# KT19/distributed-training-compare-jax

Measured on AMD Instinct MI355X. Metric: avg step time (ms) + tokens/sec, GPT-2-small DP/TP/PP at 1/2/4/8 MI355X, higher is better.
Workload: dtype bf16; 1 GPU; model=gpt2-small-124M (d768 L12 H12 F3072 T1024 V50258), global_batch=8, seq_len=1024, parallelism=dp1, capture_comms=True, hipgraph=True, backend=nccl, world_size=1, graph_segments=1, eager_collectives=0

## Files before the change

### distributed_training_compare_jax_amd/csrc/gemm.hip

```cpp
#include "common.h"
#include "gemm_plan.h"
#include <algorithm>
#include <cstdlib>
#include <type_traits>

namespace {

constexpr int NT = 256;

template <int R, int BK, bool KMAJ>
struct Tile {
  static constexpr int LD = KMAJ ? (BK + 16) : (R + 16);
  static constexpr int ROWS = KMAJ ? R : BK;
  static constexpr int ELEMS = ROWS * LD;
  static constexpr int CHUNKS = R * BK / 8;
  static constexpr int PER_THREAD = CHUNKS / NT;
  static_assert(CHUNKS % NT == 0, "tile too small for 256 threads");

  __device__ __forceinline__ static void load(u32x4 (&reg)[PER_THREAD], __amdgpu_buffer_rsrc_t rs, long ld, int r0,
                                              int k0, int tid) {
#pragma unroll
    for (int i = 0; i < PER_THREAD; ++i) {
      int c = tid + i * NT;
      long off;
// ... 1494 lines not shown
    case 3: P8_VMCNT(3); break;
    case 4: P8_VMCNT(4); break;
    case 5: P8_VMCNT(5); break;
    case 6: P8_VMCNT(6); break;
    case 8: P8_VMCNT(8); break;
    case 9: P8_VMCNT(9); break;
    case 10: P8_VMCNT(10); break;
    case 11: P8_VMCNT(11); break;
    case 12: P8_VMCNT(12); break;
    case 15: P8_VMCNT(15); break;
    case 16: P8_VMCNT(16); break;
    case 18: P8_VMCNT(18); break;
    default: P8_VMCNT(0); break;
  }
}

template <int B, int E, typename F>
__device__ __forceinline__ void static_for(F&& f) {
  if constexpr (B < E) {
    f(std::integral_constant<int, B>{});
    static_for<B + 1, E>(f);
  }
}

template <int EPI, bool OUTF32>
__device__ __forceinline__ void n8_frag_out(const Epi& e, int m, int n, f32x4 v, f32x4 bias, bf16x4 aux) {
  float o[4];
#pragma unroll
  for (int r = 0; r < 4; ++r) o[r] = v[r] + bias[r];
  if (EPI == EPI_DGELU) {
#pragma unroll
    for (int r = 0; r < 4; ++r) o[r] *= (float)aux[r];
  }
  if (OUTF32) {
    *(f32x4*)((float*)e.C + (long)m * e.ldc + n) = f32x4{o[0], o[1], o[2], o[3]};
    return;
  }
  bf16x4 ob, gb;
#pragma unroll
  for (int r = 0; r < 4; ++r) {
    if (EPI == EPI_GELU) {
      float gv, dgv;
      gelu_tanh_and_grad_f(o[r], gv, dgv);
      ob[r] = f2bf(dgv);
      gb[r] = f2bf(gv);
    } else {
      ob[r] = f2bf(o[r]);
    }
  }
  *(bf16x4*)((bf16*)e.C + (long)m * e.ldc + n) = ob;
  if (EPI == EPI_GELU) *(bf16x4*)((bf16*)e.aux_out + (long)m * e.ldc + n) = gb;
}

template <int CB, int NS, bool AK, bool BKM, int EPI, bool OUTF32>
__global__ void __launch_bounds__(NT2, 1)
gemm8n_kernel(const bf16* __restrict__ A, long lda, const bf16* __restrict__ B, long ldb, int M, int N, int K,
              int tiles_m, int tiles_n, int gm, Epi e) {
  static_assert(NS >= 3, "stage t+1 must be issued before the phase-0 wait of step t");
  constexpr int CA = 2, TM = 4, TN = CB, BN = 64 * CB, D = NS - 1, PIECES = CA + CB;
  constexpr int SIMG = PIECES * P8_CHUNK;
  __shared__ __attribute__((aligned(16))) bf16 smem[NS * SIMG];
  const int tid = threadIdx.x, lane = tid & 63, wave = tid >> 6;
  const int wr = wave >> 2, wc = wave & 3;
  const int ntiles = tiles_m * tiles_n;
  const int G = gridDim.x;
  const int bl = xcd_remap(blockIdx.x, G);
  const int nk = K / 64;
  DTC_ASSERT(nk >= 1);
  const int nr = bl < ntiles ? (ntiles - bl + G - 1) / G : 0;
  const int S = nr * nk;
  if (S == 0) return;
  auto origin = [&](int r, int& m0, int& n0) {
    const int tile = bl + r * G;
    const int grp = tile / (gm * tiles_n), in_g = tile % (gm * tiles_n);
    const int gm_eff = min(gm, tiles_m - grp * gm);
    m0 = (grp * gm + in_g % gm_eff) * 128;
    n0 = (in_g / gm_eff) * BN;
  };

  f32x4 acc[TN][TM];
#pragma unroll
  for (int i = 0; i < TN; ++i)
#pragma unroll
    for (int j = 0; j < TM; ++j) acc[i][j] = f32x4{0.f, 0.f, 0.f, 0.f};

  constexpr bool OVL = EPI == EPI_STORE || EPI == EPI_GELU;
  constexpr int NFRAG = TN * TM, NPEEL = OVL ? NFRAG / 4 : 0;
  f32x4 pacc[TN][TM], pbias[TN];
  bool pend = false;
  int em0 = 0, en0 = 0;
  const int g4e = 4 * (lane >> 4);
  auto epi_frag = [&](auto F) {
    constexpr int f = decltype(F)::value, i = f / TM, j = f % TM;
    const int m = em0 + wr * 64 + j * 16 + (lane & 15);
    const int n = en0 + wc * 16 * TN + i * 16 + g4e;
    if (m < M) n8_frag_out<EPI, OUTF32>(e, m, n, pacc[i][j], pbias[i], bf16x4{});
  };
  int cm0, cn0;
  origin(0, cm0, cn0);
  DTC_ASSERT(nk >= NPEEL);

  auto imgA = [&](int s) { return smem + (s % NS) * SIMG; };
  auto imgB = [&](int s) { return smem + (s % NS) * SIMG + CA * P8_CHUNK; };
  int pr = 0, pk = 0;
  const bf16* srcA[CA];
  const bf16* srcB[CB];
  long offA = 0, offB = 0;
  const long stepA = AK ? 64 : 64 * lda, stepB = BKM ? 64 : 64 * ldb;
  auto set_src = [&](int r) {
    int m0, n0;
    origin(r, m0, n0);
#pragma unroll
    for (int q = 0; q < CA; ++q) srcA[q] = p8_src<AK>(A, lda, m0, M, q, wave, lane);
#pragma unroll
    for (int q = 0; q < CB; ++q) srcB[q] = p8_src<BKM>(B, ldb, n0, N, q, wave, lane);
    offA = offB = 0;
  };
  set_src(0);
  auto advance = [&]() {
    offA += stepA;
    offB += stepB;
    if (++pk == nk) {
      pk = 0;
      ++pr;
      if (pr < nr) set_src(pr);
    }
  };
  auto dmaA = [&](int s, int q) { p8_dma_at(srcA[q] + offA, imgA(s), q, wave); };
  auto dmaB = [&](int s, int q) { p8_dma_at(srcB[q] + offB, imgB(s), q, wave); };

  const int npro = min(D, S);
  for (int s = 0; s < npro; ++s) {
#pragma unroll
    for (int q = 0; q < CB; ++q) dmaB(s, q);
#pragma unroll
    for (int q = 0; q < CA; ++q) dmaA(s, q);
    advance();
  }
  n8_vmcnt((npro - 1) * PIECES);
  __builtin_amdgcn_s_barrier();
  if (wr == 1) __builtin_amdgcn_s_barrier();

  int t = 0;
  bf16x8 fb[TN][2], fa[2][2];
  auto kstep = [&](auto SLc) {
    constexpr int SL = decltype(SLc)::value;
    const bf16* sA = imgA(t);
    const bf16* sB = imgB(t);
    const bool issue = t + D < S;
#pragma unroll
    for (int p = 0; p < 2; ++p) {
      if (p == 0) {
#pragma unroll
        for (int i = 0; i < TN; ++i)
#pragma unroll
          for (int kk = 0; kk < 2; ++kk) fb[i][kk] = p8_frag<BKM>(sB, TN * wc + i, kk, lane);
      }
#pragma unroll
      for (int jj = 0; jj < 2; ++jj)
#pragma unroll
        for (int kk = 0; kk < 2; ++kk) fa[jj][kk] = p8_frag<AK>(sA, 4 * wr + 2 * p + jj, kk, lane);
      if (issue) {
        if (p == 0) {
#pragma unroll
          for (int q = 0; q < CB; ++q) dmaB(t + D, q);
        } else {
#pragma unroll
          for (int q = 0; q < CA; ++q) dmaA(t + D, q);
          advance();
        }
      }
      __builtin_amdgcn_s_barrier();
      asm volatile("s_waitcnt lgkmcnt(0)" ::: "memory");
#pragma unroll
      for (int jj = 0; jj < 2; ++jj)
#pragma unroll
        for (int kk = 0; kk < 2; ++kk) asm volatile("" : "+v"(fa[jj][kk]));
#pragma unroll
      for (int i = 0; i < TN; ++i)
#pragma unroll
        for (int kk = 0; kk < 2; ++kk) asm volatile("" : "+v"(fb[i][kk]));
      __builtin_amdgcn_s_setprio(1);
#pragma unroll
      for (int kk = 0; kk < 2; ++kk)
#pragma unroll
        for (int i = 0; i < TN; ++i)
#pragma unroll
          for (int jj = 0; jj < 2; ++jj)
            acc[i][2 * p + jj] = __builtin_amdgcn_mfma_f32_16x16x32_bf16(fb[i][kk], fa[jj][kk], acc[i][2 * p + jj], 0, 0, 0);
      __builtin_amdgcn_s_setprio(0);
      if constexpr (SL >= 0) {
        if (pend) {
          if (p == 0) {
            epi_frag(std::integral_constant<int, 4 * SL>{});
            epi_frag(std::integral_constant<int, 4 * SL + 1>{});
          } else {
            epi_frag(std::integral_constant<int, 4 * SL + 2>{});
            epi_frag(std::integral_constant<int, 4 * SL + 3>{});
          }
        }
      }
      if (p == 0 && t + 1 < S) {
        if (t + D < S) {
          vmcnt_c<(D - 2) * PIECES + CB>();
        } else {
          const int full = max(0, min(t + D - 1, S - 1) - (t + 1));
          n8_vmcnt(full * PIECES);
        }
      }
      __builtin_amdgcn_s_barrier();
    }
    ++t;
  };
  for (int cr = 0; cr < nr; ++cr) {
    static_for<0, NPEEL>([&](auto sl) { kstep(sl); });
    for (int k = NPEEL; k < nk; ++k) kstep(std::integral_constant<int, -1>{});
    const int m0 = cm0, n0 = cn0;
    if (cr + 1 < nr) origin(cr + 1, cm0, cn0);
    const int g4 = 4 * (lane >> 4);
    if constexpr (OVL) {
#pragma unroll
      for (int i = 0; i < TN; ++i) {
        pbias[i] = e.bias ? *(const f32x4*)(e.bias + n0 + wc * 16 * TN + i * 16 + g4) : f32x4{0.f, 0.f, 0.f, 0.f};
#pragma unroll
        for (int j = 0; j < TM; ++j) pacc[i][j] = acc[i][j];
      }
      em0 = m0;
      en0 = n0;
      pend = true;
    } else if constexpr (EPI == EPI_NONE) {
#pragma unroll
      for (int i = 0; i < TN; ++i)
#pragma unroll
        for (int j = 0; j < TM; ++j) asm volatile("" ::"v"(acc[i][j]));
    } else {
#pragma unroll
      for (int i = 0; i < TN; ++i)
#pragma unroll
        for (int j = 0; j < TM; ++j) {
          const int m = m0 + wr * 64 + j * 16 + (lane & 15);
          const int n = n0 + wc * 16 * TN + i * 16 + g4;
          if (m < M && n < N) epilogue_store<EPI, OUTF32>(e, m, n, acc[i][j]);
        }
    }
#pragma unroll
    for (int i = 0; i < TN; ++i)
#pragma unroll
      for (int j = 0; j < TM; ++j) acc[i][j] = f32x4{0.f, 0.f, 0.f, 0.f};
  }
  if constexpr (OVL) static_for<0, NFRAG>([&](auto f) { epi_frag(f); });
  if (wr == 0) __builtin_amdgcn_s_barrier();
}

__device__ __forceinline__ bf16x8 ce_colsum_frag(const bf16* img, int r0, int vt, int lane) {
  const int g = lane >> 4, li = lane & 15, q = li >> 2, pp = li & 3;
  const int row = r0 + 4 * g + q;
  const int ch = 2 * vt + (pp >> 1);
  const bf16* p0 = img + row * 64 + ((ch ^ ((row >> 1) & 7)) << 3) + (pp & 1) * 4;
  const s16x4 lo = ds_tr16_asm(p0), hi = ds_tr16_asm(p0 + 16 * 64);
  return __builtin_bit_cast(bf16x8, __builtin_shufflevector(lo, hi, 0, 1, 2, 3, 4, 5, 6, 7));
}

struct CeDgradArgs {
  const bf16* logits; long ldl;
  const float* lse; const int* labels; int vocab_start, n_valid; float scale;
  const bf16* wt; long ldw;
  bf16* dlogits; long ldd;
  float* colpart;
  float* slab;
  int M, N, K, tiles_m, tiles_n, gm, split, kps;
};

__global__ void __launch_bounds__(NT2, 1) ce_dgrad256_kernel(CeDgradArgs a) {
  constexpr int TM = 8, TN = 4;
  __shared__ __attribute__((aligned(16))) bf16 smem[4 * IMG];
  const int tid = threadIdx.x, lane = tid & 63, wave = tid >> 6;
  const int wm = wave & 1, wn = wave >> 1;
  const int ntiles = a.tiles_m * a.tiles_n;
  const int lid = xcd_remap(blockIdx.x, ntiles * a.split);
  const int tile = lid % ntiles, z = lid / ntiles;
  const int grp = tile / (a.gm * a.tiles_n), in_g = tile % (a.gm * a.tiles_n);
  const int gm_eff = min(a.gm, a.tiles_m - grp * a.gm);
  const int tm_idx = grp * a.gm + in_g % gm_eff, tn_idx = in_g / gm_eff;
  const int m0 = tm_idx * BIG, n0 = tn_idx * BIG;
  DTC_ASSERT(tm_idx >= 0 && tn_idx >= 0 && z >= 0 && m0 < a.M && n0 < a.N);
  const int kbeg = z * a.kps;
  const int nk = min(a.kps, a.K - kbeg) / 64;
// ... 643 lines not shown
  if constexpr (V::epi == EPI_STORE && V::f32) {
    if (p.sub == 3) {
      const int tn3 = a.N / 192;
      hipLaunchKernelGGL((gemm8p_kernel<V::AK, V::BKM, V::epi, V::f32, 3>), dim3(tiles_m * tn3 * split), dim3(NT2), 0, st,
                         (const bf16*)a.A, a.lda, (const bf16*)a.B, a.ldb, a.M, a.N, a.K, tiles_m, tn3,
                         gm_round32(tiles_m, tn3), split, kps, (float*)a.workspace, e);
      DTC_CHECK_LAUNCH();
      note_launch(gp::FAM_BIG, BIG, 192, split, 3, 0, a.layout, V::epi);
      return finish_splitk(a, split, st);
    }
  }
  const int gm = tiles_n <= 16 ? gm_round32(tiles_m, tiles_n) : wide_gm(tiles_m);
  hipLaunchKernelGGL((gemm8p_kernel<V::AK, V::BKM, V::epi, V::f32>), dim3(tiles_m * tiles_n * split), dim3(NT2), 0, st,
                     (const bf16*)a.A, a.lda, (const bf16*)a.B, a.ldb, a.M, a.N, a.K, tiles_m, tiles_n, gm, split,
                     kps, (float*)a.workspace, e);
  DTC_CHECK_LAUNCH();
  note_launch(gp::FAM_BIG, BIG, BIG, split, 4, 0, a.layout, V::epi);
  return finish_splitk(a, split, st);
}

template <class V, int CB2>
int launch_r8_cb(const GemmArgs& a, const gp::GemmPlan& p, hipStream_t st) {
  const Epi e = make_epi(a, 0);
  R8Args r;
  r.A = (const bf16*)a.A; r.lda = a.lda; r.B = (const bf16*)a.B; r.ldb = a.ldb;
  r.M = a.M; r.N = a.N; r.K = a.K; r.n_split = p.aux;
  r.tm = a.M / BIG;
  r.tn1 = r.n_split / BIG;
  r.nb1 = r.tm * r.tn1;
  r.gm1 = r.tn1 > 0 ? gm_round32(r.tm, r.tn1) : 1;
  r.tn2 = (a.N - r.n_split) / (64 * CB2);
  r.gm2 = gm_round32(r.tm, std::max(1, r.tn2));
  r.ilv = g_knobs.r8_ilv && r.nb1 >= 2 && r.tm * r.tn2 >= 2;
  const int grid = r.nb1 + r.tm * r.tn2;
  hipLaunchKernelGGL((gemm8r_kernel<V::AK, V::BKM, V::epi, V::f32, CB2>), dim3(grid), dim3(NT2), 0, st, r, e);
  DTC_CHECK_LAUNCH();
  note_launch(gp::FAM_R8, BIG, 64 * CB2, 1, CB2, r.n_split, a.layout, V::epi);
  return 0;
}

template <class V>
int launch_r8(const GemmArgs& a, const gp::GemmPlan& p, hipStream_t st) {
  if (p.sub == 4) return launch_r8_cb<V, 4>(a, p, st);
  if (p.sub == 2) return launch_r8_cb<V, 2>(a, p, st);
  return launch_r8_cb<V, 1>(a, p, st);
}

template <class V, int CB>
int launch_n8_cb(const GemmArgs& a, hipStream_t st) {
  const Epi e = make_epi(a, 0);
  const int tiles_m = (a.M + 127) / 128, tiles_n = a.N / (64 * CB);
  constexpr int NS = CB == 3 ? 4 : 3;
  const int grid = std::min(tiles_m * tiles_n, cu_count());
  hipLaunchKernelGGL((gemm8n_kernel<CB, NS, V::AK, V::BKM, V::epi, V::f32>), dim3(grid), dim3(NT2), 0, st,
                     (const bf16*)a.A, a.lda, (const bf16*)a.B, a.ldb, a.M, a.N, a.K, tiles_m, tiles_n,
                     gm_n8(tiles_m, tiles_n), e);
  DTC_CHECK_LAUNCH();
  note_launch(gp::FAM_N8, 128, 64 * CB, 1, CB, 0, a.layout, V::epi);
  return 0;
}

template <class V>
int launch_n8(const GemmArgs& a, const gp::GemmPlan& p, hipStream_t st) {
  return p.sub == 3 ? launch_n8_cb<V, 3>(a, st) : launch_n8_cb<V, 4>(a, st);
}

template <class V, int CFG>
int launch_w(const GemmArgs& a, int split, hipStream_t st) {
  constexpr gp::WTile T = gp::W_TILES[CFG];
  const int tiles_m = (a.M + T.bm - 1) / T.bm, tiles_n = (a.N + T.bn - 1) / T.bn;
  const Epi e = make_epi(a, tiles_n * T.wgn);
  const int nk = a.K / 64;
  const int kps = ((nk + split - 1) / split) * 64;
  hipLaunchKernelGGL((gemm_dmaw_kernel<T.bm, T.bn, T.stages, T.wgm, T.wgn, V::AK, V::BKM, V::epi, V::f32>),
                     dim3(tiles_m * tiles_n * split), dim3(64 * T.wgm * T.wgn), 0, st, (const bf16*)a.A, a.lda,
                     (const bf16*)a.B, a.ldb, a.M, a.N, a.K, tiles_m, tiles_n, gm_xcd_share(tiles_m, tiles_n), split, kps,
                     (float*)a.workspace, e);
  DTC_CHECK_LAUNCH();
  note_launch(gp::FAM_DMAW, T.bm, T.bn, split, T.stages, T.wgm * 10 + T.wgn, a.layout, V::epi);
  return finish_splitk(a, split, st);
}

template <class V, int CFG>
int launch_w_if(const GemmArgs& a, const gp::GemmPlan& p, hipStream_t st) {
  if constexpr (gp::dmaw_cfg_has(CFG, V::layout, V::epi, V::f32))
    if (p.bm == gp::W_TILES[CFG].bm && p.bn == gp::W_TILES[CFG].bn) return launch_w<V, CFG>(a, p.split, st);
  return NOT_INSTANTIATED;
}

template <class V>
int launch_dmaw(const GemmArgs& a, const gp::GemmPlan& p, hipStream_t st) {
  int r = launch_w_if<V, gp::W_256x128>(a, p, st);
  if (r == NOT_INSTANTIATED) r = launch_w_if<V, gp::W_128x64>(a, p, st);
  if (r == NOT_INSTANTIATED) r = launch_w_if<V, gp::W_64x128>(a, p, st);
  if (r == NOT_INSTANTIATED) r = launch_w_if<V, gp::W_128x128>(a, p, st);
  return r;
}

int launch(const gp::GemmPlan& p, const GemmArgs& a, hipStream_t st) {
  return with_variant(a.layout, p.epi, p.f32, [&](auto v) {
    using V = decltype(v);
    constexpr int L = V::layout, E = V::epi;
    constexpr bool F = V::f32;
    switch (p.family) {
      case gp::FAM_R8: if constexpr (gp::r8_has(L, E, F)) return launch_r8<V>(a, p, st); break;
      case gp::FAM_N8: if constexpr (gp::n8_has(L, E, F)) return launch_n8<V>(a, p, st); break;
      case gp::FAM_DMAW: return launch_dmaw<V>(a, p, st);
      case gp::FAM_BIG: if constexpr (gp::big_has(L, E, F)) return launch_big<V>(a, p, st); break;
      case gp::FAM_REG:
// ... 123 lines not shown
  if (a->M <= 0 || a->M % 128 || a->N % 256 || a->N > 1024 || a->K <= 0 || a->K % 64) return 1400;
  if (a->lda % 8 || a->ldb % 8) return 1400;
  if (!a->sync || !a->step || !a->gamma || !a->err || !a->C || !a->y || !a->mean || !a->rstd) return 1401;
  if (a->bwd ? (!a->x || !a->part || a->nslab < 2 || a->nslab > 3) : (!a->resid || !a->beta)) return 1402;
  Epi e{};
  e.M = a->M; e.N = a->N; e.C = a->C; e.ldc = a->N; e.bias = a->bwd ? nullptr : a->bias;
  e.aux = a->resid; e.ldaux = a->N; e.alpha = 1.f;
  e.ln.gamma = a->gamma; e.ln.beta = a->beta; e.ln.y = (bf16*)a->y; e.ln.mean = a->mean; e.ln.rstd = a->rstd;
  e.ln.x = a->x; e.ln.part = a->part; e.ln.nslab = a->nslab; e.ln.eps = a->eps;
  e.ln.sync = a->sync; e.ln.step = a->step; e.ln.site = a->site; e.ln.nsites = a->nsites; e.ln.err = a->err;
  const int tiles_m = a->M / 128, tiles_n = a->N / 64;
  const dim3 grid(tiles_m * tiles_n), block(512);
  if (a->bwd)
    hipLaunchKernelGGL((gemm_dmaw_kernel<128, 64, 4, 4, 2, true, true, EPI_LN_BWD, true>), grid, block, 0, st,
                       (const bf16*)a->A, a->lda, (const bf16*)a->B, a->ldb, a->M, a->N, a->K, tiles_m, tiles_n, tiles_m,
                       1, a->K, nullptr, e);
  else
    hipLaunchKernelGGL((gemm_dmaw_kernel<128, 64, 4, 4, 2, true, true, EPI_RESID_LN, true>), grid, block, 0, st,
                       (const bf16*)a->A, a->lda, (const bf16*)a->B, a->ldb, a->M, a->N, a->K, tiles_m, tiles_n, tiles_m,
                       1, a->K, nullptr, e);
  DTC_CHECK_LAUNCH();
  note_launch(gp::FAM_LN, 128, 64, 1, a->bwd ? 1 : 0, 0, 0, a->bwd ? EPI_LN_BWD : EPI_RESID_LN);
  return 0;
}

long dtc_gemm_ln_sync_words(int M, int N) { return (long)M * (N / 32) + (long)(M / 128) * (N / 64); }

int dtc_lmhead_nparts(int M, int N, int K) {
  const gp::GemmPlan p = plan_query(0, M, N, K, EPI_LMHEAD, false, false);
  if (p.bn == BIG || gp::big_split(0, M, N, K, g_knobs)) return ((N + 255) / 256) * 4;
  return ((N + 127) / 128) * 2;
}

int dtc_gemm_wgrad_split(int M, int N, int K, int has_db) {
  return plan_query(2, M, N, K, EPI_STORE, true, has_db != 0).split;
}

int dtc_gemm_wgrad_fuses_colsum(int M, int N, int K) {
  return plan_query(2, M, N, K, EPI_STORE, true, true).err != 1009;
}

long dtc_gemm_workspace_bytes(int layout, int M, int N, int K) {
  const int bs = gp::big_split(layout, M, N, K, g_knobs);
  int split = bs ? bs : gp::reg_plan(M, N, K, layout == 2 ? 1 : (layout == 1 ? 2 : 0), g_knobs).split;
  if (layout == 2 && !bs) split = std::max(split, gp::dmaw_plan(2, M, N, K, EPI_STORE, true, false, g_knobs).split);
  return split > 1 ? (long)split * M * N * 4 : 0;
}

int dtc_gemm_set_wgrad256(int on) { return set_knob(g_knobs.wgrad256, on); }
int dtc_gemm_set_n8(int mask) { return set_knob(g_knobs.n8_mask, mask); }
int dtc_gemm_set_big_cb3(int on) { return set_knob(g_knobs.big_cb3, on); }
int dtc_gemm_set_n8_mink(int k) { return set_knob(g_knobs.n8_mink, k); }
int dtc_gemm_set_n8_cb(int cb) { return set_knob(g_knobs.n8_cb, cb); }
int dtc_gemm_set_r8(int mask) { return set_knob(g_knobs.r8_mask, mask); }
int dtc_gemm_set_r8_ilv(int on) { return set_knob(g_knobs.r8_ilv, on); }

int dtc_wg_entry_bytes() { return (int)sizeof(WgEntry); }
int dtc_wg_max() { return WG_MAX; }
int dtc_wg_batch_bytes() { return (int)sizeof(WgBatch); }

int dtc_wgrad_group(const WgBatch* in, hipStream_t st) {
  DTC_HOST_CHECK(in && in->n >= 1 && in->n <= WG_MAX && in->K >= 64 && in->K % 64 == 0);
  WgBatch b = *in;
  int t = 0;
  for (int i = 0; i < b.n; ++i) {
    WgEntry& w = b.e[i];
    DTC_HOST_CHECK(w.A && w.B && w.C && w.M >= 8 && w.N >= 8 && w.M % 8 == 0 && w.N % 8 == 0);
    DTC_HOST_CHECK(((unsigned long)w.A % 16) == 0 && ((unsigned long)w.B % 16) == 0 && ((unsigned long)w.C % 16) == 0);
    w.tile0 = t;
    t += ((w.M + BIG - 1) / BIG) * ((w.N + BIG - 1) / BIG);
    w.nfast = g_knobs.wg_nfast && w.M >= 2 * w.N;
  }
  b.ntiles = t;
  int tail = 0, split = 0;
  const int cus = cu_count();
  if (in->tail_slab && in->tail_split > 0 && cus > 0 && t > cus) {
    tail = t % cus;
    split = in->tail_split > 1 ? in->tail_split : std::max(2, std::min(4, tail > 0 ? cus / tail : 0));
    bool ok = tail > 0 && b.K % (64 * split) == 0 && (long)tail * split <= 2L * cus &&
              (long)tail * split * BIG * BIG <= in->tail_cap;
    for (int i = 0; ok && i < b.n; ++i) {
      const WgEntry& w = b.e[i];
      const int end = w.tile0 + ((w.M + BIG - 1) / BIG) * ((w.N + BIG - 1) / BIG);
      if (end > t - tail && w.cs) ok = false;
    }
    if (!ok) tail = split = 0;
  }
  b.tail_tiles = tail;
  b.tail_split = split > 1 ? split : 1;
  if (!tail) b.tail_slab = nullptr;
  hipLaunchKernelGGL(gemm8p_group_kernel, dim3(t - tail + tail * b.tail_split), dim3(NT2), 0, st, b);
  DTC_CHECK_LAUNCH();
  note_launch(gp::FAM_WGROUP, BIG, BIG, b.tail_split, tail, t, 2, EPI_STORE);
  if (tail) {
    hipLaunchKernelGGL(wg_tail_reduce, dim3(tail * 8), dim3(WGT_THREADS), 0, st, b);
    DTC_CHECK_LAUNCH();
  }
  return 0;
}

int dtc_gemm_last_launch(int* out) {
  const LastLaunch l = g_last;
  out[0] = l.family; out[1] = l.bm; out[2] = l.bn; out[3] = l.split;
  out[4] = l.sub; out[5] = l.aux; out[6] = l.layout; out[7] = l.epi;
  return 0;
}
// ... 3 lines not shown
```

### distributed_training_compare_jax_amd/csrc/gemm_plan.h

```cpp
#pragma once
#include <algorithm>
#include <climits>
#include <cstdlib>

namespace gp {

enum { EPI_STORE = 0, EPI_RESID = 1, EPI_GELU = 2, EPI_DGELU = 3, EPI_LMHEAD = 4, EPI_LMHEAD_EVAL = 7 };
constexpr int BIG = 256;

enum {
  FAM_NONE = 0,
  FAM_REG = 1,
  FAM_DMA64 = 2,
  FAM_DMAW = 3,
  FAM_BIG = 4,
  FAM_R8 = 5,
  FAM_N8 = 6,
  FAM_PAIR = 7,
  FAM_WGROUP = 8,
  FAM_CE_DGRAD = 9,
  FAM_LN = 10,
  FAM_COUNT = 11,
};

struct Knobs {
  int dma_fwd64 = 1;
  int wgrad_blocks_128 = 256;
  int wgrad_blocks_64 = 512;
  int wide_gm = 3;
  int wgrad_cs256 = 1;
  int wgrad256 = 1;
  int gemm256 = 7;
  int big_min_tiles = 512;
  int big_tail = 64;
  int big_cb3 = 1;
  int r8_mask = 5;
  int r8_ilv = 1;
  int n8_mask = 3;
  int n8_cb = 0;
  int n8_mink = 1024;
  int w8_mode = 1;
  int wg_nfast = 1;
};

inline int env_int(const char* value, int dflt) { return value ? atoi(value) : dflt; }

inline Knobs knobs_from_env() {
  Knobs k;
  k.dma_fwd64 = env_int(getenv("DTC_GEMM_DMA"), k.dma_fwd64);
  k.wgrad_blocks_128 = env_int(getenv("DTC_WGRAD_BLOCKS"), k.wgrad_blocks_128);
  k.wgrad_blocks_64 = env_int(getenv("DTC_WGRAD_BLOCKS"), k.wgrad_blocks_64);
  k.wide_gm = env_int(getenv("DTC_WIDE_GM"), k.wide_gm);
  k.wgrad_cs256 = env_int(getenv("DTC_WGRAD_CS256"), k.wgrad_cs256);
  k.wgrad256 = env_int(getenv("DTC_WGRAD256"), k.wgrad256);
  k.gemm256 = env_int(getenv("DTC_GEMM256"), k.gemm256);
  k.big_min_tiles = env_int(getenv("DTC_BIG_MIN_TILES"), k.big_min_tiles);
  k.big_tail = env_int(getenv("DTC_BIG_TAIL"), k.big_tail);
  k.big_cb3 = env_int(getenv("DTC_BIG_CB3"), k.big_cb3);
  k.r8_mask = env_int(getenv("DTC_GEMM8R"), k.r8_mask);
  k.r8_ilv = env_int(getenv("DTC_R8_ILV"), k.r8_ilv);
  k.n8_mask = env_int(getenv("DTC_GEMM8N"), k.n8_mask);
  k.n8_cb = env_int(getenv("DTC_N8_CB"), k.n8_cb);
  k.n8_mink = env_int(getenv("DTC_N8_MINK"), k.n8_mink);
  k.w8_mode = env_int(getenv("DTC_GEMM_W8"), k.w8_mode);
  k.wg_nfast = env_int(getenv("DTC_WG_NFAST"), k.wg_nfast);
  return k;
}

struct Problem {
  int layout, M, N, K;
  int epi;
  bool f32;
  bool has_bias, has_colsum;
  bool unit_ab;
  bool eval_ok;
  long ws_bytes;
};

struct GemmPlan {
  int err = 0;
  int family = FAM_NONE;
  int bm = 0, bn = 0;
  int bk = 64;
  int split = 1;
  int sub = 0, aux = 0;
  int epi = 0;
  bool f32 = false;
};

inline GemmPlan reg_plan(int M, int N, int K, int allow_split, const Knobs& k) {
  GemmPlan p;
  p.family = FAM_REG;
  p.bm = p.bn = 128;
  if (K % 64) {
    p.bm = p.bn = 64;
    p.bk = 32;
    return p;
  }
  const int nk = K / 64;
  const long t128 = (long)((M + 127) / 128) * ((N + 127) / 128);
  if (allow_split && K >= 8192 && t128 >= 32) {
    p.split = (int)std::max(1L, std::min((long)nk / 64, (512 + t128 - 1) / t128));
    return p;
  }
  if (allow_split == 1 && t128 < 256) {
    while (t128 * p.split < k.wgrad_blocks_128 && nk / (p.split * 2) >= 8) p.split *= 2;
    return p;
  }
  if (t128 >= 256) return p;
  p.bm = p.bn = 64;
  const long t64 = (long)((M + 63) / 64) * ((N + 63) / 64);
  if (allow_split == 1)
    while (t64 * p.split < k.wgrad_blocks_64 && nk / (p.split * 2) >= 4) p.split *= 2;
  return p;
}

// ... 263 lines not shown
```

### distributed_training_compare_jax_amd/models/gpt.py

```python

from __future__ import annotations

import contextlib
from dataclasses import dataclass
from typing import Dict, Optional, Tuple

import torch

from ..config.schema import ModelConfig
from ..ops import attention as A
from ..ops import embedding as E
from ..ops import gemm as G
from ..ops import layernorm as LN
from ..ops import fp8 as F8
from ..ops import mxfp8 as MX
from ..ops import ln_fused as LF
from ..ops import xent as X
from ..ops.reduce import GradReducer
from .params import head_split
from ..parallel.buffers import FlatParams


import os as _os

_CE_FUSED_MODE = _os.environ.get("DTC_CE_FUSED", "auto")


def _ce_fused(tokens: int, d: int) -> bool:
    if _CE_FUSED_MODE == "auto":
        return tokens * d <= 4096 * 512
    return _CE_FUSED_MODE == "1"
_CE_CHUNK = int(_os.environ.get("DTC_CE_CHUNK", "0"))
_ADD_LN = _os.environ.get("DTC_ADD_LN", "1") == "1"
_FWD_BF16 = _os.environ.get("DTC_FWD_BF16", "0") == "1"
_RED_BATCH_LAYERS = _os.environ.get("DTC_RED_BATCH_LAYERS", "1") == "1"
if _CE_CHUNK < 0 or _CE_CHUNK % 256:
    raise ValueError(f"DTC_CE_CHUNK={_CE_CHUNK}: must be 0 (off) or a positive multiple of 256 vocab columns")



_HEAD_BF16_MAXK = 16384


class _Staged:

    __slots__ = ("rows", "cols", "device")

    def __init__(self, rows: int, cols: int, device):
        self.rows, self.cols, self.device = rows, cols, device

class NoComm:

    size = 1
    rank = 0

    def all_reduce_(self, t):
        return t

    def all_gather_stack(self, t):
        return t.unsqueeze(0)


@dataclass
class StageLayout:
    layers: range
    has_embed: bool
    has_head: bool
    head_part: Tuple[int, int] = (0, 1)


class GPTStage:

    def __init__(self, cfg: ModelConfig, flat: FlatParams, layout: StageLayout, tp=None,
                 dropout_seed: int = 0, act_dtype: torch.dtype = torch.bfloat16):
        self.cfg = cfg
        dev = torch.device(flat.device)
        layer_bytes = 4 * (4 * cfg.d_model * cfg.d_model + 2 * cfg.d_model * cfg.d_ff)
        self.red = GradReducer(dev, arena_mb=max(512, (32 * layer_bytes // 3) >> 20)) if dev.type == "cuda" else None
        self._bias_fused = set()
        self.param_ready: Dict = {}
        self.flat = flat
        self.layout = layout
        self.tp = tp if tp is not None else NoComm()
        self.seed = int(dropout_seed)
        self.act_dtype = act_dtype
        D, H = cfg.d_model, cfg.n_heads
# ... 183 lines not shown
            y1q = MX.quant_mxfp8(y1)
        qkv = MX.linear_mxfp8(y1q, f.wmx(p + "qkv.w"), f.p(p + "qkv.b"), out_dtype=act)
        o, lse = A.attn_fwd(qkv.view(batch, T, -1), self.heads_local)
        o = o.view(batch * T, -1)
        oq = MX.quant_mxfp8(o)
        if _ADD_LN:
            br = MX.linear_mxfp8(oq, f.wmx(p + "out.w"), f.p(p + "out.b"), out_dtype=self._branch_dtype)
            x2, (y2, mu2, rs2), y2q = MX.add_layernorm_fwd_mx(br, x, f.p(p + "ln2.g"), f.p(p + "ln2.b"), self.eps, act)
        else:
            x2 = MX.linear_resid_mxfp8(oq, f.wmx(p + "out.w"), f.p(p + "out.b"), x)
            (y2, mu2, rs2), y2q = MX.layernorm_fwd_mx(x2, f.p(p + "ln2.g"), f.p(p + "ln2.b"), self.eps, act)
        u, gact, gq = MX.linear_gelu_mxfp8(y2q, f.wmx(p + "fc1.w"), f.p(p + "fc1.b"), out_dtype=act, quant_out=True)
        nxt = f"h.{l + 1}.ln1" if (l + 1) in self.layout.layers else ("lnf" if self.layout.has_head else None)
        if _ADD_LN and nxt is not None:
            br = MX.linear_mxfp8(gq, f.wmx(p + "fc2.w"), f.p(p + "fc2.b"), out_dtype=self._branch_dtype)
            if nxt == "lnf":
                x3, ctx["lnf_pre"] = LN.add_layernorm_fwd(br, x2, f.p("lnf.g"), f.p("lnf.b"), self.eps, act)
            else:
                x3, ctx[("ln1", l + 1)], ctx[("ln1_mx", l + 1)] = MX.add_layernorm_fwd_mx(
                    br, x2, f.p(nxt + ".g"), f.p(nxt + ".b"), self.eps, act)
        else:
            x3 = MX.linear_resid_mxfp8(gq, f.wmx(p + "fc2.w"), f.p(p + "fc2.b"), x2)
        ctx[l] = (x, y1, mu1, rs1, qkv, o, lse, x2, y2, mu2, rs2, u, gact, batch)
        return x3

    def block_forward(self, l: int, x: torch.Tensor, batch: int, ctx: Dict) -> torch.Tensor:
        if self.sp:
            return self._block_forward_sp(l, x, batch, ctx)
        if self.mx:
            return self._block_forward_mx(l, x, batch, ctx)
        self._await_params(l)
        f, p = self.flat, f"h.{l}."
        tp = self.tp
        lead = tp.rank == 0
        T = x.shape[0] // batch
        pre = ctx.pop(("ln1", l), None)
        if pre is None:
            pre = LN.layernorm_fwd(x, f.p(p + "ln1.g"), f.p(p + "ln1.b"), self.eps, self.act_dtype)
        y1, mu1, rs1 = pre
        fp8 = self.fp8
        if fp8:
            qkv = F8.linear_fp8(F8.quant_e4m3(y1), f.w8(p + "qkv.w"), f.p(p + "qkv.b"), out_dtype=self.act_dtype)
        else:
            qkv = G.linear(y1, f.w(p + "qkv.w"), f.p(p + "qkv.b"))
        o, lse = A.attn_fwd(qkv.view(batch, T, -1), self.heads_local)
        o = o.view(batch * T, -1)
        oq = F8.quant_e4m3(o) if fp8 else None
        if self._fuse_fwd:
            x2, (y2, mu2, rs2) = LF.linear_resid_ln(o, f.w(p + "out.w"), f.p(p + "out.b"), x, f.p(p + "ln2.g"),
                                                    f.p(p + "ln2.b"), self.eps, self.ln_sync, self._ln_site(l, 0, False))
        elif self.tp_bf16:
            x2 = self._row_parallel(o, p + "out.w", resid=x, bias=f.p(p + "out.b"))
            y2, mu2, rs2 = LN.layernorm_fwd(x2, f.p(p + "ln2.g"), f.p(p + "ln2.b"), self.eps, self.act_dtype)
        elif tp.size == 1 and _ADD_LN:
            br = (F8.linear_fp8(oq, f.w8(p + "out.w"), f.p(p + "out.b"), out_dtype=self._branch_dtype) if fp8 else
                  G.linear(o, f.w(p + "out.w"), f.p(p + "out.b"), out_dtype=self._branch_dtype))
            x2, (y2, mu2, rs2) = LN.add_layernorm_fwd(br, x, f.p(p + "ln2.g"), f.p(p + "ln2.b"), self.eps,
                                                      self.act_dtype)
        else:
            if fp8:
                x2 = F8.linear_resid_fp8(oq, f.w8(p + "out.w"), f.p(p + "out.b"), x)
            else:
                x2 = G.linear_resid(o, f.w(p + "out.w"), f.p(p + "out.b") if lead else None, x if lead else None)
            tp.all_reduce_(x2)
            y2, mu2, rs2 = LN.layernorm_fwd(x2, f.p(p + "ln2.g"), f.p(p + "ln2.b"), self.eps, self.act_dtype)
        if fp8:
            u, gact = F8.linear_gelu_fp8(F8.quant_e4m3(y2), f.w8(p + "fc1.w"), f.p(p + "fc1.b"), out_dtype=self.act_dtype)
            gq = F8.quant_e4m3(gact)
        else:
            u, gact = G.linear_gelu(y2, f.w(p + "fc1.w"), f.p(p + "fc1.b"))
        nxt = f"h.{l + 1}.ln1" if (l + 1) in self.layout.layers else ("lnf" if self.layout.has_head else None)
        if self._fuse_fwd and nxt is not None:
            x3, pre_next = LF.linear_resid_ln(gact, f.w(p + "fc2.w"), f.p(p + "fc2.b"), x2, f.p(nxt + ".g"),
                                              f.p(nxt + ".b"), self.eps, self.ln_sync, self._ln_site(l, 1, False))
            ctx[("ln1", l + 1) if nxt != "lnf" else "lnf_pre"] = pre_next
        elif tp.size == 1 and _ADD_LN and nxt is not None and not self.tp_bf16:
            br = (F8.linear_fp8(gq, f.w8(p + "fc2.w"), f.p(p + "fc2.b"), out_dtype=self._branch_dtype) if fp8 else
                  G.linear(gact, f.w(p + "fc2.w"), f.p(p + "fc2.b"), out_dtype=self._branch_dtype))
            x3, pre_next = LN.add_layernorm_fwd(br, x2, f.p(nxt + ".g"), f.p(nxt + ".b"), self.eps, self.act_dtype)
            ctx[("ln1", l + 1) if nxt != "lnf" else "lnf_pre"] = pre_next
        elif self.tp_bf16:
            x3 = self._row_parallel(gact, p + "fc2.w", resid=x2, bias=f.p(p + "fc2.b"))
        elif fp8:
            x3 = F8.linear_resid_fp8(gq, f.w8(p + "fc2.w"), f.p(p + "fc2.b"), x2)
        else:
            x3 = G.linear_resid(gact, f.w(p + "fc2.w"), f.p(p + "fc2.b") if lead else None, x2 if lead else None)
            tp.all_reduce_(x3)
        ctx[l] = (x, y1, mu1, rs1, qkv, o, lse, x2, y2, mu2, rs2, u, gact, batch)
        return x3

    def block_backward(self, l: int, ctx: Dict, dx3: torch.Tensor, dx3_c: torch.Tensor, beta: float, dx_hook=None):
        if self.sp:
            return self._block_backward_sp(l, ctx, dx3, dx3_c, beta, dx_hook)
        f, p = self.flat, f"h.{l}."
        x, y1, mu1, rs1, qkv, o, lse, x2, y2, mu2, rs2, u, gact, batch = ctx.pop(l)
        T = x.shape[0] // batch
        red = self.red
        fc2b_fused = l in self._bias_fused
        self._bias_fused.discard(l)
        self._beta = beta
        if self._defer_wg:
            wt2 = f.wt(p + "fc2.w")
            du = (G.matmul_nt_dgelu(dx3_c, wt2, u) if wt2 is not None
                  else G.matmul_nn_dgelu(dx3_c, f.w(p + "fc2.w"), u))
            self._wg(dx3_c, gact, p + "fc2")
            if not fc2b_fused:
                G.colsum(dx3, f.g(p + "fc2.b"), beta, red=red)
        else:
            du = G.linear_backward(dx3_c, f.w(p + "fc2.w"), gact, f.g(p + "fc2.w"), beta, red=red, dgelu_u=u,
                                   wt=f.wt(p + "fc2.w"))
            if not fc2b_fused:
                G.colsum(dx3, f.g(p + "fc2.b"), beta, red=red)
        wt1 = f.wt(p + "fc1.w")
        if self._fuse_bwd and wt1 is not None:
            dx2, dx2_c = LF.dgrad_ln_bwd(du, wt1, x2, f.p(p + "ln2.g"), mu2, rs2, dx3, f.g(p + "ln2.g"),
                                         f.g(p + "ln2.b"), beta, dbias=f.g(p + "out.b"), red=red,
                                         sync=self.ln_sync, site=self._ln_site(l, 0, True))
            self._wg(du, y2, p + "fc1", bias=True)
        else:
            dy2 = self._tp_reduce(self._dgrad_wgrad(du, p + "fc1", y2, beta, red, pair=False))
            dx2, dx2_c = self._ln_bwd(dy2, x2, p + "ln2", mu2, rs2, dx3, beta, bias_grad=p + "out.b")
        wto = f.wt(p + "out.w")
        if wto is not None:
            do = G.linear(dx2_c, wto)
            self._wg(dx2_c, o, p + "out")
        elif self._defer_wg:
            do = G.matmul_nn(dx2_c, f.w(p + "out.w"), out_dtype=self.act_dtype)
            self._wg(dx2_c, o, p + "out")
        else:
# ... 423 lines not shown
```

### distributed_training_compare_jax_amd/ops/_native.py

```python

from __future__ import annotations

import ctypes
import os
import threading

import torch

_LIB = None
_LOCK = threading.Lock()
LIB_NAME = "_dtc_kernels.so"
PKG_DIR = os.path.dirname(os.path.dirname(os.path.abspath(__file__)))
LIB_PATH = os.environ.get("DTC_KERNEL_LIB") or os.path.join(PKG_DIR, LIB_NAME)

c_int = ctypes.c_int
c_long = ctypes.c_long
c_float = ctypes.c_float
c_vp = ctypes.c_void_p


class GemmArgs(ctypes.Structure):

    _fields_ = [
        ("layout", c_int),
# ... 29 lines not shown
        ("C", c_vp),
        ("bias", c_vp), ("resid", c_vp), ("gamma", c_vp), ("beta", c_vp),
        ("y", c_vp), ("mean", c_vp), ("rstd", c_vp),
        ("x", c_vp), ("part", c_vp), ("nslab", c_int),
        ("eps", c_float),
        ("sync", c_vp), ("step", c_vp), ("site", c_int), ("nsites", c_int),
        ("err", c_vp),
    ]


class WgEntry(ctypes.Structure):

    _fields_ = [("A", c_vp), ("B", c_vp), ("C", c_vp), ("cs", c_vp), ("M", c_int), ("N", c_int),
                ("tile0", c_int), ("nfast", c_int)]


WG_MAX = 64


class WgBatch(ctypes.Structure):
    _fields_ = [("n", c_int), ("K", c_int), ("beta", c_float), ("ntiles", c_int), ("sq", c_vp),
                ("tail_tiles", c_int), ("tail_split", c_int), ("tail_slab", c_vp), ("tail_cap", c_long),
                ("e", WgEntry * WG_MAX)]


EPI_STORE = 0
EPI_RESID = 1
EPI_GELU = 2
EPI_DGELU = 3
EPI_LMHEAD = 4
EPI_LMHEAD_EVAL = 7


def _declare(lib):
    vp, i, l, f = c_vp, c_int, c_long, c_float
    sigs = {
        "dtc_version": ([], i),
        "dtc_gemm": ([ctypes.POINTER(GemmArgs), vp], i),
        "dtc_gemm_workspace_bytes": ([i, i, i, i], l),
        "dtc_lmhead_nparts": ([i, i, i], i),
        "dtc_layernorm_fwd": ([vp, vp, vp, vp, vp, vp, i, i, f, i, vp], i),
        "dtc_add_layernorm_fwd": ([vp, vp, vp, vp, vp, vp, vp, vp, i, i, f, i, vp], i),
        "dtc_add_layernorm_fwd_bf16": ([vp, vp, vp, vp, vp, vp, vp, vp, i, i, f, i, vp], i),
        "dtc_layernorm_bwd": ([vp, i, vp, vp, vp, vp, vp, vp, vp, vp, vp, vp, i, i, i, vp, l, i, vp], i),
        "dtc_layernorm_bwd_workspace_bytes": ([i, i], l),
        "dtc_colsum": ([vp, i, i, i, l, vp, f, vp, l, i, vp], i),
        "dtc_gemm_wgrad_split": ([i, i, i, i], i),
        "dtc_gemm_set_n8": ([i], i),
        "dtc_gemm_set_n8_cb": ([i], i),
        "dtc_gemm_set_r8": ([i], i),
        "dtc_gemm_set_r8_ilv": ([i], i),
        "dtc_gemm_set_big_cb3": ([i], i),
        "dtc_gemm_set_n8_mink": ([i], i),
        "dtc_gemm_set_wgrad256": ([i], i),
        "dtc_gemm_last_launch": ([ctypes.POINTER(c_int)], i),
        "dtc_wgrad_group": ([ctypes.POINTER(WgBatch), vp], i),
        "dtc_wg_entry_bytes": ([], i),
        "dtc_wg_max": ([], i),
        "dtc_wg_batch_bytes": ([], i),
        "dtc_gemm_pair": ([ctypes.POINTER(GemmArgs), ctypes.POINTER(GemmArgs), vp], i),
        "dtc_gemm_ln": ([ctypes.POINTER(LnArgs), vp], i),
        "dtc_gemm_ln_sync_words": ([i, i], l),
        "dtc_gemm_wgrad_fuses_colsum": ([i, i, i], i),
        "dtc_reduce_tasks": ([vp, vp], i),
        "dtc_red_max_tasks": ([], i),
        "dtc_red_task_bytes": ([], i),
        "dtc_colsum_workspace_bytes": ([i, i], l),
        "dtc_embed_fwd": ([vp, vp, vp, vp, i, i, i, i, f, l, vp, l, vp], i),
        "dtc_epoch_inc": ([vp, vp], i),
        "dtc_flag_set": ([vp, i, vp, vp], i),
        "dtc_flag_wait": ([vp, i, vp, vp, vp], i),
        "dtc_p2p_flag_bytes": ([], l),
        "dtc_p2p_alloc": ([l, vp, vp], i),
        "dtc_p2p_open": ([vp, vp], i),
        "dtc_p2p_close": ([vp], i),
        "dtc_device_pci_bus_id": ([i, ctypes.c_char_p, i], i),
        "dtc_device_count": ([ctypes.POINTER(c_int)], i),
        "dtc_graph_num_nodes": ([c_vp, ctypes.POINTER(ctypes.c_size_t)], i),
        "dtc_can_access_peer": ([i, i, ctypes.POINTER(c_int)], i),
        "dtc_p2p_free": ([vp], i),
        "dtc_p2p_allreduce": ([vp, vp, l, vp, i, i, l, vp, vp, i, vp], i),
        "dtc_p2p_allreduce_bf16": ([vp, vp, l, vp, i, i, l, vp, vp, i, vp, vp, i, vp], i),
        "dtc_p2p_barrier_round": ([vp, i, i, vp, vp, vp], i),
        "dtc_p2p_reduce_scatter": ([vp, i, vp, l, vp, i, i, l, vp, vp, vp, vp, i, vp], i),
        "dtc_p2p_all_gather": ([vp, vp, l, vp, i, i, l, vp, vp, vp], i),
        "dtc_dp_allreduce": ([vp, l, i, vp, i, i, l, vp, vp, i, vp], i),
        "dtc_dp_rs_slots": ([l, i, i, i], i),
        "dtc_dp_reduce_scatter": ([vp, l, i, vp, i, vp, i, i, l, vp, vp, i, vp], i),
        "dtc_dp_param_gather": ([vp, vp, l, l, i, vp, i, i, l, vp, vp, i, vp], i),
        "dtc_pp_send": ([vp, l, vp, l, l, vp, i, vp, vp], i),
        "dtc_pp_recv": ([vp, vp, l, vp, l, l, vp, i, vp, vp, vp], i),
        "dtc_cu_hog": ([i, l, i, vp, vp], i),
        "dtc_embed_sort_bits": ([i], i),
        "dtc_embed_sort": ([vp, i, i, vp, vp], i),
        "dtc_embed_bwd": ([vp, vp, vp, vp, vp, i, i, i, i, f, l, vp, l, i, vp, vp, i, vp], i),
        "dtc_embed_sq_slots": ([i, i, i], l),
        "dtc_attn_fwd": ([vp, vp, vp, i, i, i, i, l, f, vp], i),
        "dtc_attn_bwd": ([vp, vp, vp, vp, vp, i, i, i, i, i, f, vp, l, vp], i),
        "dtc_attn_bwd_workspace_bytes": ([i, i, i, i], l),
        "dtc_ce_combine": ([vp, i, i, l, l, vp, vp, vp, f, vp, i, vp], i),
        "dtc_ce_eval_finish": ([vp, l, l, vp, i, l, l, i, i, i, vp, vp, vp, vp, vp, vp], i),
        "dtc_row_argmax_f32": ([vp, l, i, i, vp, vp, vp], i),
        "dtc_ce_bwd": ([vp, l, vp, vp, i, i, i, i, f, vp, vp], i),
        "dtc_ce_colsum_rows": ([], i),
        "dtc_sumsq_segments": ([vp, vp, i, vp, vp, vp, l, vp], i),
        "dtc_sumsq_workspace_bytes": ([], l),
# ... 84 lines not shown
```

Baseline: 791,800 tokens/s.

## Prefetch fp32 residual during GEMM k-loop and route unfused residual via linear_resid

Adds a PRE variant of the n8 GEMM kernel for the fp32 residual epilogue. The residual tile and bias are loaded into registers during the first k-steps of each tile, with vmcnt waits adjusted to account for the extra loads, so the epilogue no longer stalls on global reads. It also changes the default DTC_ADD_LN handling so that, for bf16 non-fp8 runs, the separate add+layernorm path is skipped in favour of the linear_resid path that uses this epilogue. The cost is higher register pressure from holding the residual fragments, plus a change in which forward kernels run by default.

```diff
diff --git a/distributed_training_compare_jax_amd/csrc/gemm.hip b/distributed_training_compare_jax_amd/csrc/gemm.hip
--- a/distributed_training_compare_jax_amd/csrc/gemm.hip
+++ b/distributed_training_compare_jax_amd/csrc/gemm.hip
@@ -1570,7 +1570,15 @@
   if (EPI == EPI_GELU) *(bf16x4*)((bf16*)e.aux_out + (long)m * e.ldc + n) = gb;
 }
 
-template <int CB, int NS, bool AK, bool BKM, int EPI, bool OUTF32>
+template <int NLD, int D>
+constexpr int n8_rpre_younger(int sl) {
+  int c = 0;
+  for (int s = sl - (D - 1); s <= sl; ++s)
+    if (s >= 0 && s < NLD) c += (s == sl || s == sl - (D - 1)) ? 2 : 4;
+  return c;
+}
+
+template <int CB, int NS, bool AK, bool BKM, int EPI, bool OUTF32, bool PRE = false>
 __global__ void __launch_bounds__(NT2, 1)
 gemm8n_kernel(const bf16* __restrict__ A, long lda, const bf16* __restrict__ B, long ldb, int M, int N, int K,
               int tiles_m, int tiles_n, int gm, Epi e) {
@@ -1603,8 +1611,11 @@
     for (int j = 0; j < TM; ++j) acc[i][j] = f32x4{0.f, 0.f, 0.f, 0.f};
 
   constexpr bool OVL = EPI == EPI_STORE || EPI == EPI_GELU;
-  constexpr int NFRAG = TN * TM, NPEEL = OVL ? NFRAG / 4 : 0;
-  f32x4 pacc[TN][TM], pbias[TN];
+  constexpr bool RPRE = PRE && EPI == EPI_RESID && OUTF32;
+  static_assert(RPRE == PRE, "PRE is the fp32 residual epilogue's");
+  constexpr int NFRAG = TN * TM, NLD = NFRAG / 4;
+  constexpr int NPEEL = OVL ? NLD : RPRE ? NLD + D - 1 : 0;
+  f32x4 pacc[TN][TM], pbias[TN], rpre[TN][TM];
   bool pend = false;
   int em0 = 0, en0 = 0;
   const int g4e = 4 * (lane >> 4);
@@ -1617,6 +1628,19 @@
   int cm0, cn0;
   origin(0, cm0, cn0);
   DTC_ASSERT(nk >= NPEEL);
+  auto rpre_load = [&](auto F) {
+    constexpr int f = decltype(F)::value, i = f / TM, j = f % TM;
+    const int m = min(cm0 + wr * 64 + j * 16 + (lane & 15), M - 1);
+    const int n = cn0 + wc * 16 * TN + i * 16 + g4e;
+    DTC_ASSERT(m >= 0 && n >= 0 && n + 4 <= N);
+    rpre[i][j] = *(const f32x4*)((const float*)e.aux + (long)m * e.ldaux + n);
+  };
+  auto rpre_bias = [&]() {
+#pragma unroll
+    for (int i = 0; i < TN; ++i)
+      pbias[i] = e.bias ? *(const f32x4*)(e.bias + cn0 + wc * 16 * TN + i * 16 + g4e) : f32x4{0.f, 0.f, 0.f, 0.f};
+  };
+  if constexpr (RPRE) rpre_bias();
 
   auto imgA = [&](int s) { return smem + (s % NS) * SIMG; };
   auto imgB = [&](int s) { return smem + (s % NS) * SIMG + CA * P8_CHUNK; };
@@ -1688,6 +1712,15 @@
           advance();
         }
       }
+      if constexpr (RPRE && SL >= 0 && SL < NLD) {
+        if (p == 0) {
+          rpre_load(std::integral_constant<int, 4 * SL>{});
+          rpre_load(std::integral_constant<int, 4 * SL + 1>{});
+        } else {
+          rpre_load(std::integral_constant<int, 4 * SL + 2>{});
+          rpre_load(std::integral_constant<int, 4 * SL + 3>{});
+        }
+      }
       __builtin_amdgcn_s_barrier();
       asm volatile("s_waitcnt lgkmcnt(0)" ::: "memory");
 #pragma unroll
@@ -1707,7 +1740,7 @@
           for (int jj = 0; jj < 2; ++jj)
             acc[i][2 * p + jj] = __builtin_amdgcn_mfma_f32_16x16x32_bf16(fb[i][kk], fa[jj][kk], acc[i][2 * p + jj], 0, 0, 0);
       __builtin_amdgcn_s_setprio(0);
-      if constexpr (SL >= 0) {
+      if constexpr (OVL && SL >= 0) {
         if (pend) {
           if (p == 0) {
             epi_frag(std::integral_constant<int, 4 * SL>{});
@@ -1720,7 +1753,7 @@
       }
       if (p == 0 && t + 1 < S) {
         if (t + D < S) {
-          vmcnt_c<(D - 2) * PIECES + CB>();
+          vmcnt_c<(D - 2) * PIECES + CB + (RPRE && SL >= 0 ? n8_rpre_younger<NLD, D>(SL) : 0)>();
         } else {
           const int full = max(0, min(t + D - 1, S - 1) - (t + 1));
           n8_vmcnt(full * PIECES);
@@ -1751,6 +1784,24 @@
       for (int i = 0; i < TN; ++i)
 #pragma unroll
         for (int j = 0; j < TM; ++j) asm volatile("" ::"v"(acc[i][j]));
+    } else if constexpr (RPRE) {
+#pragma unroll
+      for (int i = 0; i < TN; ++i) {
+        const int n = n0 + wc * 16 * TN + i * 16 + g4;
+#pragma unroll
+        for (int j = 0; j < TM; ++j) {
+          const int m = m0 + wr * 64 + j * 16 + (lane & 15);
+          f32x4 o;
+#pragma unroll
+          for (int r = 0; r < 4; ++r) {
+            o[r] = e.alpha * acc[i][j][r] + pbias[i][r];
+            o[r] += rpre[i][j][r];
+          }
+          asm volatile("" : "+v"(o));
+          if (m < M) DTC_OUT_STORE((f32x4*)((float*)e.C + (long)m * e.ldc + n), o);
+        }
+      }
+      if (cr + 1 < nr) rpre_bias();
     } else {
 #pragma unroll
       for (int i = 0; i < TN; ++i)
@@ -2500,9 +2551,16 @@
   const int tiles_m = (a.M + 127) / 128, tiles_n = a.N / (64 * CB);
   constexpr int NS = CB == 3 ? 4 : 3;
   const int grid = std::min(tiles_m * tiles_n, cu_count());
-  hipLaunchKernelGGL((gemm8n_kernel<CB, NS, V::AK, V::BKM, V::epi, V::f32>), dim3(grid), dim3(NT2), 0, st,
-                     (const bf16*)a.A, a.lda, (const bf16*)a.B, a.ldb, a.M, a.N, a.K, tiles_m, tiles_n,
-                     gm_n8(tiles_m, tiles_n), e);
+  constexpr bool RESID = V::epi == EPI_RESID && V::f32;
+  if (RESID && g_knobs.n8_rpre && a.K / 64 >= CB + NS - 2) {
+    hipLaunchKernelGGL((gemm8n_kernel<CB, NS, V::AK, V::BKM, V::epi, V::f32, RESID>), dim3(grid), dim3(NT2), 0, st,
+                       (const bf16*)a.A, a.lda, (const bf16*)a.B, a.ldb, a.M, a.N, a.K, tiles_m, tiles_n,
+                       gm_n8(tiles_m, tiles_n), e);
+  } else {
+    hipLaunchKernelGGL((gemm8n_kernel<CB, NS, V::AK, V::BKM, V::epi, V::f32>), dim3(grid), dim3(NT2), 0, st,
+                       (const bf16*)a.A, a.lda, (const bf16*)a.B, a.ldb, a.M, a.N, a.K, tiles_m, tiles_n,
+                       gm_n8(tiles_m, tiles_n), e);
+  }
   DTC_CHECK_LAUNCH();
   note_launch(gp::FAM_N8, 128, 64 * CB, 1, CB, 0, a.layout, V::epi);
   return 0;
@@ -2732,6 +2790,7 @@
 int dtc_gemm_set_big_cb3(int on) { return set_knob(g_knobs.big_cb3, on); }
 int dtc_gemm_set_n8_mink(int k) { return set_knob(g_knobs.n8_mink, k); }
 int dtc_gemm_set_n8_cb(int cb) { return set_knob(g_knobs.n8_cb, cb); }
+int dtc_gemm_set_n8_rpre(int on) { return set_knob(g_knobs.n8_rpre, on); }
 int dtc_gemm_set_r8(int mask) { return set_knob(g_knobs.r8_mask, mask); }
 int dtc_gemm_set_r8_ilv(int on) { return set_knob(g_knobs.r8_ilv, on); }
 
diff --git a/distributed_training_compare_jax_amd/csrc/gemm_plan.h b/distributed_training_compare_jax_amd/csrc/gemm_plan.h
--- a/distributed_training_compare_jax_amd/csrc/gemm_plan.h
+++ b/distributed_training_compare_jax_amd/csrc/gemm_plan.h
@@ -39,6 +39,7 @@
   int n8_mask = 3;
   int n8_cb = 0;
   int n8_mink = 1024;
+  int n8_rpre = 1;
   int w8_mode = 1;
   int wg_nfast = 1;
 };
@@ -62,6 +63,7 @@
   k.n8_mask = env_int(getenv("DTC_GEMM8N"), k.n8_mask);
   k.n8_cb = env_int(getenv("DTC_N8_CB"), k.n8_cb);
   k.n8_mink = env_int(getenv("DTC_N8_MINK"), k.n8_mink);
+  k.n8_rpre = env_int(getenv("DTC_N8_RPRE"), k.n8_rpre);
   k.w8_mode = env_int(getenv("DTC_GEMM_W8"), k.w8_mode);
   k.wg_nfast = env_int(getenv("DTC_WG_NFAST"), k.wg_nfast);
   return k;
diff --git a/distributed_training_compare_jax_amd/models/gpt.py b/distributed_training_compare_jax_amd/models/gpt.py
--- a/distributed_training_compare_jax_amd/models/gpt.py
+++ b/distributed_training_compare_jax_amd/models/gpt.py
@@ -31,7 +31,14 @@
         return tokens * d <= 4096 * 512
     return _CE_FUSED_MODE == "1"
 _CE_CHUNK = int(_os.environ.get("DTC_CE_CHUNK", "0"))
-_ADD_LN = _os.environ.get("DTC_ADD_LN", "1") == "1"
+def _add_ln_sites(value: str):
+    if value not in ("0", "1", "out", "fc2"):
+        raise ValueError(f"DTC_ADD_LN={value!r}: expected 0, 1, out or fc2")
+    return value in ("1", "out"), value in ("1", "fc2")
+
+
+_ADD_LN_OUT, _ADD_LN_FC2 = _add_ln_sites(_os.environ.get("DTC_ADD_LN", "0"))
+_ADD_LN = _os.environ.get("DTC_ADD_LN", "1") != "0"
 _FWD_BF16 = _os.environ.get("DTC_FWD_BF16", "0") == "1"
 _RED_BATCH_LAYERS = _os.environ.get("DTC_RED_BATCH_LAYERS", "1") == "1"
 if _CE_CHUNK < 0 or _CE_CHUNK % 256:
@@ -321,7 +328,7 @@
         elif self.tp_bf16:
             x2 = self._row_parallel(o, p + "out.w", resid=x, bias=f.p(p + "out.b"))
             y2, mu2, rs2 = LN.layernorm_fwd(x2, f.p(p + "ln2.g"), f.p(p + "ln2.b"), self.eps, self.act_dtype)
-        elif tp.size == 1 and _ADD_LN:
+        elif tp.size == 1 and _ADD_LN and (fp8 or _FWD_BF16 or _ADD_LN_OUT):
             br = (F8.linear_fp8(oq, f.w8(p + "out.w"), f.p(p + "out.b"), out_dtype=self._branch_dtype) if fp8 else
                   G.linear(o, f.w(p + "out.w"), f.p(p + "out.b"), out_dtype=self._branch_dtype))
             x2, (y2, mu2, rs2) = LN.add_layernorm_fwd(br, x, f.p(p + "ln2.g"), f.p(p + "ln2.b"), self.eps,
@@ -343,7 +350,8 @@
             x3, pre_next = LF.linear_resid_ln(gact, f.w(p + "fc2.w"), f.p(p + "fc2.b"), x2, f.p(nxt + ".g"),
                                               f.p(nxt + ".b"), self.eps, self.ln_sync, self._ln_site(l, 1, False))
             ctx[("ln1", l + 1) if nxt != "lnf" else "lnf_pre"] = pre_next
-        elif tp.size == 1 and _ADD_LN and nxt is not None and not self.tp_bf16:
+        elif (tp.size == 1 and _ADD_LN and (fp8 or _FWD_BF16 or _ADD_LN_FC2) and nxt is not None
+              and not self.tp_bf16):
             br = (F8.linear_fp8(gq, f.w8(p + "fc2.w"), f.p(p + "fc2.b"), out_dtype=self._branch_dtype) if fp8 else
                   G.linear(gact, f.w(p + "fc2.w"), f.p(p + "fc2.b"), out_dtype=self._branch_dtype))
             x3, pre_next = LN.add_layernorm_fwd(br, x2, f.p(nxt + ".g"), f.p(nxt + ".b"), self.eps, self.act_dtype)
diff --git a/distributed_training_compare_jax_amd/ops/_native.py b/distributed_training_compare_jax_amd/ops/_native.py
--- a/distributed_training_compare_jax_amd/ops/_native.py
+++ b/distributed_training_compare_jax_amd/ops/_native.py
@@ -105,6 +105,7 @@
         "dtc_gemm_set_r8_ilv": ([i], i),
         "dtc_gemm_set_big_cb3": ([i], i),
         "dtc_gemm_set_n8_mink": ([i], i),
+        "dtc_gemm_set_n8_rpre": ([i], i),
         "dtc_gemm_set_wgrad256": ([i], i),
         "dtc_gemm_last_launch": ([ctypes.POINTER(c_int)], i),
         "dtc_wgrad_group": ([ctypes.POINTER(WgBatch), vp], i),
```

Measured after the change: 795,400 tokens/s, median of 6. About the same (+0.5%).
